# psklavos1/NeRF-Sys

Measured on AMD Instinct MI355X. Metric: rays/sec (train step) + full-image PSNR, 800×800 Lego, 64+128 samples, higher is better.
Workload: dtype f32; 1 GPU; Lego-style 800x800 (synthetic analytic scene, 100 views), 64 coarse + 128 fine hierarchical, 2 x (8x256 MLP), fp32, train step incl. ray gen + Adam [fused engine]; global_batch=4096, rays_per_gpu=4096, parallelism=dp1, precision=fp32, fp32_gemm=split, full=False

## Files before the change

nerf-sys_amd/csrc/gemm_x6.hpp:

```cpp
#pragma once
#include "gemm_bf16.hpp"

typedef float x6_f32x2 __attribute__((ext_vector_type(2)));
typedef __bf16 x6_bf16x2 __attribute__((ext_vector_type(2)));
typedef float x6_f32x4 __attribute__((ext_vector_type(4)));
__device__ __forceinline__ uint32_t x6_pack(float a, float b) {
  return __builtin_bit_cast(uint32_t, __builtin_convertvector(x6_f32x2{a, b}, x6_bf16x2));
}

__device__ __forceinline__ void x6_split4(const float4 v, uint2& h, uint2& m, uint2& l) {
  const uint32_t h0 = x6_pack(v.x, v.y), h1 = x6_pack(v.z, v.w);
  const float r0 = v.x - nerf_bf16_lo(h0), r1 = v.y - nerf_bf16_hi(h0);
  const float r2 = v.z - nerf_bf16_lo(h1), r3 = v.w - nerf_bf16_hi(h1);
  const uint32_t m0 = x6_pack(r0, r1), m1 = x6_pack(r2, r3);
  const uint32_t l0 = x6_pack(r0 - nerf_bf16_lo(m0), r1 - nerf_bf16_hi(m0));
  const uint32_t l1 = x6_pack(r2 - nerf_bf16_lo(m1), r3 - nerf_bf16_hi(m1));
  h = make_uint2(h0, h1);
  m = make_uint2(m0, m1);
  l = make_uint2(l0, l1);
}

__device__ constexpr int X6_PA[6] = {2, 1, 0, 1, 0, 0};
__device__ constexpr int X6_PB[6] = {0, 1, 2, 0, 1, 0};
#define X6_MFMA_BLOCK(acc_, TM_, TN_, FIRST_, SECOND_)                                                      \
  _Pragma("unroll") for (int t_ = 0; t_ < 6; ++t_)                                                        \
    _Pragma("unroll") for (int a_ = 0; a_ < TM_; ++a_)                                                    \
      _Pragma("unroll") for (int b_ = 0; b_ < TN_; ++b_)                                                  \
        acc_[a_][b_] = __builtin_amdgcn_mfma_f32_32x32x16_bf16(FIRST_, SECOND_, acc_[a_][b_], 0, 0, 0);

struct X6Job {
  const float* src;
  nerf_bf16* dst;
  int rows, cols, lds, transpose;
  int64_t plane;
};
struct X6Jobs {
  X6Job j[16];
};
static __global__ void x6_planes_kernel(X6Jobs jobs) {
  const X6Job J = jobs.j[blockIdx.z];
  __shared__ float tile[32][33];
  const int r0 = blockIdx.y * 32, c0 = blockIdx.x * 32;
  if (r0 >= J.rows || c0 >= J.cols) return;
  const int tx = threadIdx.x & 31, ty = threadIdx.x >> 5;
  for (int y = ty; y < 32; y += 8) {
    const int r = r0 + y, c = c0 + tx;
    tile[y][tx] = (r < J.rows && c < J.cols) ? J.src[(int64_t)r * J.lds + c] : 0.f;
  }
  __syncthreads();
  for (int y = ty; y < 32; y += 8) {
    const float v = J.transpose ? tile[tx][y] : tile[y][tx];
    const int orow = J.transpose ? c0 + y : r0 + y, ocol = J.transpose ? r0 + tx : c0 + tx;
    const int orows = J.transpose ? J.cols : J.rows, ocols = J.transpose ? J.rows : J.cols;
    if (orow < orows && ocol < ocols) {
      const nerf_bf16 h = (nerf_bf16)v;
      const float r1 = v - (float)h;
      const nerf_bf16 m = (nerf_bf16)r1;
      const nerf_bf16 l = (nerf_bf16)(r1 - (float)m);
      const int64_t o = (int64_t)orow * ocols + ocol;
      J.dst[o] = h;
      J.dst[J.plane + o] = m;
      J.dst[2 * J.plane + o] = l;
    }
  }
}


constexpr int X6E_PITCH = 36;
constexpr int X6E_WAVE_FLOATS = 32 * X6E_PITCH;
template <int TM, int TN, int EPI>
__device__ __forceinline__ void x6_epilogue_lds(nerf_f32x16 (&acc)[TM][TN], int64_t mw, int n0, int lane,
                                                const float* __restrict__ bias, float* __restrict__ C, int ldc,
                                                const uint32_t* __restrict__ mbits, int ldmb,
                                                uint32_t* __restrict__ mbits_out, float* E) {
  const int li = lane & 31, lh = lane >> 5;
  const int rr = lane >> 3, cc = 4 * (lane & 7);
#pragma unroll
  for (int b = 0; b < TN; ++b) {
    const int nb = n0 + b * 32;
    const int g = nb >> 5;
    float4 bv[4];
#pragma unroll
    for (int q = 0; q < 4; ++q) {
      bv[q] = make_float4(0.f, 0.f, 0.f, 0.f);
      if (EPI == EPI_BIAS || EPI == EPI_BIAS_RELU) bv[q] = *reinterpret_cast<const float4*>(bias + nb + 8 * q + 4 * lh);
    }
#pragma unroll
    for (int a = 0; a < TM; ++a) {
      const int64_t m = mw + a * 32 + li;
      uint32_t word = 0;
      if (EPI == EPI_MASK) word = mbits[m * ldmb + g];
#pragma unroll
      for (int q = 0; q < 4; ++q) {
        float v[4];
#pragma unroll
        for (int e = 0; e < 4; ++e) {
          v[e] = acc[a][b][4 * q + e];
          const float bb = e == 0 ? bv[q].x : (e == 1 ? bv[q].y : (e == 2 ? bv[q].z : bv[q].w));
          if (EPI == EPI_BIAS) v[e] += bb;
          if (EPI == EPI_BIAS_RELU) {
            v[e] = fmaxf(v[e] + bb, 0.f);
            word |= (v[e] > 0.f ? 1u : 0u) << (8 * q + 4 * lh + e);
          }
          if (EPI == EPI_MASK) v[e] = ((word >> (8 * q + 4 * lh + e)) & 1u) ? v[e] : 0.f;
        }
        *reinterpret_cast<float4*>(E + li * X6E_PITCH + 8 * q + 4 * lh) = make_float4(v[0], v[1], v[2], v[3]);
      }
      if (EPI == EPI_BIAS_RELU && mbits_out) {
        word |= __shfl_xor(word, 32, 64);
        if (lh == 0) mbits_out[m * ldmb + g] = word;
      }
      float4 o[4];
#pragma unroll
      for (int i = 0; i < 4; ++i) o[i] = *reinterpret_cast<const float4*>(E + (rr + 8 * i) * X6E_PITCH + cc);
#pragma unroll
      for (int i = 0; i < 4; ++i)
        *reinterpret_cast<float4*>(C + (mw + a * 32 + rr + 8 * i) * ldc + nb + cc) = o[i];
    }
  }
}

template <int EPI, bool BIGSMALL, int NKC, int TN>
__global__ __launch_bounds__(512, 1) void gemm_nt_x6w_kernel(const float* __restrict__ A, int lda,
                                                             const nerf_bf16* __restrict__ Bp, int ldb, int64_t bplane,
                                                             const float* __restrict__ bias, float* __restrict__ C,
                                                             int ldc, const uint32_t* __restrict__ mbits, int ldmb,
                                                             uint32_t* __restrict__ mbits_out, int K, int n_ntiles) {
  constexpr int BK = 32, NW = 8, TM = 1;
  constexpr int WTM = 32 * TM, BM = WTM * NW, BN = 32 * TN;
  constexpr int KS = BK / 16;
  constexpr int LS = BK;
  static_assert(BK == 32, "the swizzle assumes four 16-B chunks per row");
  auto sw = [](int r, int q) { return q ^ ((r >> 2) & 3); };
  constexpr int PL = BN * LS;
  static_assert(2 * 3 * PL >= NW * X6E_WAVE_FLOATS * 2, "epilogue tiles");
  __shared__ __attribute__((aligned(16))) nerf_bf16 smem[2 * 3 * PL];

  const int tile = xcd_remap(blockIdx.x, gridDim.x);
  const int mt = tile / n_ntiles, nt = tile - mt * n_ntiles;
  const int64_t m0 = (int64_t)mt * BM;
  const int n0 = nt * BN;
  const int tid = threadIdx.x, lane = tid & 63, wave = tid >> 6;
  const int li = lane & 31, lh = lane >> 5;
  const nerf_bf16* Bb = Bp + (int64_t)n0 * ldb;
  const float* At = A + (m0 + wave * WTM) * lda;
  int aoff[TM];
#pragma unroll
  for (int a = 0; a < TM; ++a) aoff[a] = (a * 32 + li) * lda + 8 * lh;

  constexpr bool A3 = NKC > 0;
  float4 ra[A3 ? 3 : 2][TM][KS][2];
  constexpr int GPP = BN * BK * 2 / 1024, GPW = 3 * GPP / NW;
  static_assert(GPW * NW == 3 * GPP && GPP * 1024 == BN * BK * 2, "weight staging");
  const int wave_u = __builtin_amdgcn_readfirstlane(tid >> 6);
  const uint32_t gofs = (uint32_t)((((lane >> 2) * ldb) + 8 * ((lane & 3) ^ ((lane >> 4) & 3))) * 2);
  const uint32_t smem_u32 = (uint32_t)(uintptr_t)(const __attribute__((address_space(3))) char*)smem;
#define X6W_ALOAD(set_, k0_)                                                                              \
  _Pragma("unroll") for (int a = 0; a < TM; ++a)                                                         \
    _Pragma("unroll") for (int ks = 0; ks < KS; ++ks)                                                    \
      _Pragma("unroll") for (int hf = 0; hf < 2; ++hf)                                                   \
        ra[set_][a][ks][hf] = *reinterpret_cast<const float4*>(At + aoff[a] + (k0_) + 16 * ks + 4 * hf);
  constexpr int BPG = 2;
#define X6W_BLOAD(k0_, dbuf_)                                                                             \
  {                                                                                                       \
    _Pragma("unroll") for (int a = 0; a < TM; ++a)                                                       \
      _Pragma("unroll") for (int ks = 0; ks < KS; ++ks)                                                  \
        asm volatile("" ::"v"(__builtin_bit_cast(x6_f32x4, ra[j][a][ks][0])),                            \
                     "v"(__builtin_bit_cast(x6_f32x4, ra[j][a][ks][1])) : "memory");                     \
    _Pragma("unroll") for (int i = 0; i < GPW; ++i) {                                                    \
      const int g_ = wave_u + NW * i, p_ = g_ / GPP, rb_ = (g_ % GPP) * 16;                              \
      const nerf_bf16* sb_ = Bb + p_ * bplane + (int64_t)rb_ * ldb + (k0_);                              \
      const uint32_t dst_ = smem_u32 + (uint32_t)((((dbuf_) * 3 + p_) * PL + rb_ * LS) * 2);             \
// ... 129 lines not shown
  constexpr int PG = ((BN + 127) / 128) * 128 + 32, PX = ((BK + 127) / 128) * 128 + 32;
  constexpr int IG = MR * PG, IX = MR * PX;
  constexpr int STAGE = 3 * (IG + IX);
  constexpr int G_F4 = MR * BN / 4, X_F4 = MR * BK / 4;
  constexpr int G_PER = (G_F4 + 255) / 256, X_PER = (X_F4 + 255) / 256;
  __shared__ __attribute__((aligned(16))) nerf_bf16 smem[2 * STAGE];

  const int lin = xcd_remap(blockIdx.x, gridDim.x);
  const int s = lin / n_tiles;
  const int tile = lin - s * n_tiles;
  const int nt = tile / n_ktiles, kt = tile - nt * n_ktiles;
  const int n0 = nt * BN, k0 = kt * BK;
  const int64_t r0 = (int64_t)s * rows_per_split;
  int64_t r1 = r0 + rows_per_split;
  if (r1 > M) r1 = M;
  const int tid = threadIdx.x, lane = tid & 63, wave = tid >> 6;
  const int wn = wave / WAVES_K, wk = wave % WAVES_K;
  const int li = lane & 31, lh = lane >> 5;
  const bool do_bias = (Pb != nullptr) && kt == 0 && wk == 0;

  constexpr int PF = 4;
  float4 rg[PF][G_PER], rx[PF][X_PER];
#define WX6_GLOAD(set_, m_)                                                                                \
  {                                                                                                        \
    _Pragma("unroll") for (int i = 0; i < G_PER; ++i) {                                                    \
      const int f = tid + 256 * i;                                                                         \
      if (G_F4 % 256 == 0 || f < G_F4)                                                                     \
        rg[set_][i] = *reinterpret_cast<const float4*>(G + ((m_) + f / (BN / 4)) * ldg + n0 + (f % (BN / 4)) * 4); \
    }                                                                                                      \
    _Pragma("unroll") for (int i = 0; i < X_PER; ++i) {                                                    \
      const int f = tid + 256 * i;                                                                         \
      if (X_F4 % 256 == 0 || f < X_F4)                                                                     \
        rx[set_][i] = *reinterpret_cast<const float4*>(X + ((m_) + f / (BK / 4)) * ldx + k0 + (f % (BK / 4)) * 4); \
    }                                                                                                      \
  }
#define WX6_SSTORE(set_, buf_)                                                                             \
  {                                                                                                        \
    nerf_bf16* Gs_ = smem + (buf_) * STAGE;                                                                \
    nerf_bf16* Xs_ = Gs_ + 3 * IG;                                                                         \
    _Pragma("unroll") for (int i = 0; i < G_PER; ++i) {                                                    \
      const int f = tid + 256 * i;                                                                         \
      if (G_F4 % 256 == 0 || f < G_F4) {                                                                   \
        uint2 h, m, l;                                                                                     \
        x6_split4(rg[set_][i], h, m, l);                                                                   \
        const int o = (f / (BN / 4)) * PG + (f % (BN / 4)) * 4;                                            \
        *reinterpret_cast<uint2*>(Gs_ + o) = h;                                                            \
        *reinterpret_cast<uint2*>(Gs_ + IG + o) = m;                                                       \
        *reinterpret_cast<uint2*>(Gs_ + 2 * IG + o) = l;                                                   \
      }                                                                                                    \
    }                                                                                                      \
    _Pragma("unroll") for (int i = 0; i < X_PER; ++i) {                                                    \
      const int f = tid + 256 * i;                                                                         \
      if (X_F4 % 256 == 0 || f < X_F4) {                                                                   \
        uint2 h, m, l;                                                                                     \
        x6_split4(rx[set_][i], h, m, l);                                                                   \
        const int o = (f / (BK / 4)) * PX + (f % (BK / 4)) * 4;                                            \
        *reinterpret_cast<uint2*>(Xs_ + o) = h;                                                            \
        *reinterpret_cast<uint2*>(Xs_ + IX + o) = m;                                                       \
        *reinterpret_cast<uint2*>(Xs_ + 2 * IX + o) = l;                                                   \
      }                                                                                                    \
    }                                                                                                      \
  }

  nerf_f32x16 acc[TM][TN];
#pragma unroll
  for (int a = 0; a < TM; ++a)
#pragma unroll
    for (int b = 0; b < TN; ++b)
#pragma unroll
      for (int r = 0; r < 16; ++r) acc[a][b][r] = 0.f;
  float bsum[TM];
#pragma unroll
  for (int a = 0; a < TM; ++a) bsum[a] = 0.f;

  const int grp = lane >> 4, q = (lane >> 2) & 3, p4 = lane & 3;
  const int trow = 8 * (grp >> 1) + q, tcol = 16 * (grp & 1) + 4 * p4;
  auto tr_frag = [&](const nerf_bf16* base, int pitch) {
    const nerf_s16x4 lo = __builtin_amdgcn_ds_read_tr16_b64_v4i16((__attribute__((address_space(3))) nerf_s16x4*)(base));
    const nerf_s16x4 hi =
        __builtin_amdgcn_ds_read_tr16_b64_v4i16((__attribute__((address_space(3))) nerf_s16x4*)(base + 4 * pitch));
    const short v8 __attribute__((ext_vector_type(8))) = {lo[0], lo[1], lo[2], lo[3], hi[0], hi[1], hi[2], hi[3]};
    return __builtin_bit_cast(nerf_bf16x8, v8);
  };

  const int64_t nit = (r1 - r0) / MR;
  if (nit > 0) {
#pragma unroll
    for (int j = 0; j < PF; ++j) WX6_GLOAD(j, r0 + (j < nit ? j : nit - 1) * MR);
    WX6_SSTORE(0, 0);
  }
  __syncthreads();
  for (int64_t it0 = 0; it0 < nit; it0 += PF) {
#pragma unroll
   for (int j = 0; j < PF; ++j) {
    const int64_t it = it0 + j;
    if (it >= nit) break;
    WX6_GLOAD(j, r0 + (it + PF < nit ? it + PF : nit - 1) * MR);
    const nerf_bf16* Gs = smem + (j & 1) * STAGE;
    const nerf_bf16* Xs = Gs + 3 * IG;
    nerf_bf16x8 af[TM][3], bf[TN][3];
#pragma unroll
    for (int pc = 0; pc < 3; ++pc) {
#pragma unroll
      for (int a = 0; a < TM; ++a) af[a][pc] = tr_frag(Gs + pc * IG + trow * PG + wn * WTN + a * 32 + tcol, PG);
#pragma unroll
      for (int b = 0; b < TN; ++b) bf[b][pc] = tr_frag(Xs + pc * IX + trow * PX + wk * WTK + b * 32 + tcol, PX);
    }
    if (do_bias) {
#pragma unroll
      for (int a = 0; a < TM; ++a)
        {
          float t8 = 0.f;
#pragma unroll
          for (int j = 0; j < 8; ++j) t8 += ((float)af[a][0][j] + (float)af[a][1][j]) + (float)af[a][2][j];
          bsum[a] += t8;
        }
    }
    WX6_SSTORE((j + 1) % PF, (j + 1) & 1);
    X6_MFMA_BLOCK(acc, TM, TN, af[a_][X6_PA[t_]], bf[b_][X6_PB[t_]])
#pragma unroll
    for (int q = 0; q < 6 * TM * TN; ++q) {
      __builtin_amdgcn_sched_group_barrier(0x008, 1, 0);
      __builtin_amdgcn_sched_group_barrier(0x002, 5, 0);
      __builtin_amdgcn_sched_group_barrier(0x200, 1, 0);
    }
    __syncthreads();
   }
  }
#undef WX6_GLOAD
#undef WX6_SSTORE

  float* Ps = P + (int64_t)s * slab;
#pragma unroll
  for (int a = 0; a < TM; ++a) {
#pragma unroll
    for (int b = 0; b < TN; ++b) {
      const int k = k0 + wk * WTK + b * 32 + li;
#pragma unroll
      for (int r = 0; r < 16; ++r) {
        const int n = n0 + wn * WTN + a * 32 + (r & 3) + 8 * (r >> 2) + 4 * lh;
        Ps[(int64_t)n * ldp + k] = acc[a][b][r];
      }
    }
  }
  if (do_bias) {
#pragma unroll
    for (int a = 0; a < TM; ++a) {
      const float v = bsum[a] + __shfl_xor(bsum[a], 32, 64);
      if (lh == 0) Pb[(int64_t)s * slab + n0 + wn * WTN + a * 32 + li] = v;
    }
  }
}

__global__ __launch_bounds__(512, 1) void gemm_wgrad_x6w_kernel(const float* __restrict__ G, int ldg,
                                                               const float* __restrict__ X, int ldx,
                                                               float* __restrict__ P, int ldp, float* __restrict__ Pb,
                                                               int64_t slab, int64_t rows_per_split, int64_t M) {
  constexpr int MR = 16, TM = 2, TN = 4, WTN = 64, WTK = 128;
  constexpr int PT = 256 + 32;
  constexpr int IMG = MR * PT;
  constexpr int STAGE = 6 * IMG;
  __shared__ __attribute__((aligned(16))) nerf_bf16 smem[2 * STAGE];

  const int s = blockIdx.x;
  const int64_t r0 = (int64_t)s * rows_per_split;
  int64_t r1 = r0 + rows_per_split;
  if (r1 > M) r1 = M;
  const int tid = threadIdx.x, lane = tid & 63, wave = tid >> 6;
  const int wn = wave >> 1, wk = wave & 1;
  const int li = lane & 31, lh = lane >> 5;
  const bool braw = Pb != nullptr;
  float4 b4 = make_float4(0.f, 0.f, 0.f, 0.f);

  constexpr int PF = 2;
  float4 rg[PF][2], rx[PF][2];
#define WX6W_GLOAD(set_, m_)                                                                               \
  _Pragma("unroll") for (int i = 0; i < 2; ++i) {                                                          \
    const int f = tid + 512 * i;                                                                           \
    rg[set_][i] = *reinterpret_cast<const float4*>(G + ((m_) + (f >> 6)) * ldg + 4 * (f & 63));            \
    rx[set_][i] = *reinterpret_cast<const float4*>(X + ((m_) + (f >> 6)) * ldx + 4 * (f & 63));            \
  }
#define WX6W_SSTORE(set_, buf_)                                                                            \
  _Pragma("unroll") for (int i = 0; i < 2; ++i) {                                                          \
    const int f = tid + 512 * i;                                                                           \
    const int o = (f >> 6) * PT + 4 * (f & 63);                                                            \
    nerf_bf16* S_ = smem + (buf_) * STAGE;                                                                 \
    uint2 h, m, l;                                                                                         \
    x6_split4(rg[set_][i], h, m, l);                                                                       \
    *reinterpret_cast<uint2*>(S_ + o) = h;                                                                 \
    *reinterpret_cast<uint2*>(S_ + IMG + o) = m;                                                           \
    *reinterpret_cast<uint2*>(S_ + 2 * IMG + o) = l;                                                       \
    x6_split4(rx[set_][i], h, m, l);                                                                       \
    *reinterpret_cast<uint2*>(S_ + 3 * IMG + o) = h;                                                       \
    *reinterpret_cast<uint2*>(S_ + 4 * IMG + o) = m;                                                       \
    *reinterpret_cast<uint2*>(S_ + 5 * IMG + o) = l;                                                       \
  }
#define WX6W_BACC(set_, sc_)                                                                               \
  _Pragma("unroll") for (int i = 0; i < 2; ++i) {                                                          \
    b4.x = fmaf(rg[set_][i].x, (sc_), b4.x);                                                               \
    b4.y = fmaf(rg[set_][i].y, (sc_), b4.y);                                                               \
    b4.z = fmaf(rg[set_][i].z, (sc_), b4.z);                                                               \
    b4.w = fmaf(rg[set_][i].w, (sc_), b4.w);                                                               \
  }

  nerf_f32x16 acc[TM][TN];
#pragma unroll
  for (int a = 0; a < TM; ++a)
#pragma unroll
    for (int b = 0; b < TN; ++b)
#pragma unroll
      for (int r = 0; r < 16; ++r) acc[a][b][r] = 0.f;
  const int grp = lane >> 4, q = (lane >> 2) & 3, p4 = lane & 3;
  const int trow = 8 * (grp >> 1) + q, tcol = 16 * (grp & 1) + 4 * p4;
  auto tr_frag = [&](const nerf_bf16* base) {
    const nerf_s16x4 lo = __builtin_amdgcn_ds_read_tr16_b64_v4i16((__attribute__((address_space(3))) nerf_s16x4*)(base));
    const nerf_s16x4 hi =
        __builtin_amdgcn_ds_read_tr16_b64_v4i16((__attribute__((address_space(3))) nerf_s16x4*)(base + 4 * PT));
    const short v8 __attribute__((ext_vector_type(8))) = {lo[0], lo[1], lo[2], lo[3], hi[0], hi[1], hi[2], hi[3]};
    return __builtin_bit_cast(nerf_bf16x8, v8);
  };

  const int64_t nit = (r1 - r0) / MR;
  if (nit > 0) {
#pragma unroll
    for (int j = 0; j < PF; ++j) WX6W_GLOAD(j, r0 + (j < nit ? j : nit - 1) * MR);
    WX6W_SSTORE(0, 0);
    if (braw) WX6W_BACC(0, 1.f);
  }
  __syncthreads();
  auto do_slab = [&](auto J, const int64_t it) __attribute__((always_inline)) {
      constexpr int j = decltype(J)::value;
      WX6W_GLOAD(j, r0 + (it + PF < nit ? it + PF : nit - 1) * MR);
      const int buf = j;
      const nerf_bf16* Gs = smem + buf * STAGE;
      const nerf_bf16* Xs = Gs + 3 * IMG;
      nerf_bf16x8 af[TM][3];
#pragma unroll
      for (int pc = 0; pc < 3; ++pc)
#pragma unroll
        for (int a = 0; a < TM; ++a) af[a][pc] = tr_frag(Gs + pc * IMG + trow * PT + wn * WTN + a * 32 + tcol);
#pragma unroll
      for (int bp = 0; bp < TN / 2; ++bp) {
        if (bp == 1) WX6W_SSTORE((j + 1) % PF, buf ^ 1);
        if (bp == 1 && braw) WX6W_BACC((j + 1) % PF, it + 1 < nit ? 1.f : 0.f);
        nerf_bf16x8 bf[2][3];
#pragma unroll
        for (int pc = 0; pc < 3; ++pc)
#pragma unroll
          for (int b = 0; b < 2; ++b)
            bf[b][pc] = tr_frag(Xs + pc * IMG + trow * PT + wk * WTK + (2 * bp + b) * 32 + tcol);
#pragma unroll
        for (int t = 0; t < 6; ++t)
#pragma unroll
          for (int a = 0; a < TM; ++a)
#pragma unroll
            for (int b = 0; b < 2; ++b)
              acc[a][2 * bp + b] = __builtin_amdgcn_mfma_f32_32x32x16_bf16(af[a][X6_PA[t]], bf[b][X6_PB[t]],
                                                                         acc[a][2 * bp + b], 0, 0, 0);
        if (bp == 1) {
          __builtin_amdgcn_sched_group_barrier(0x100, 6, 0);
#pragma unroll
          for (int q = 0; q < 24; ++q) {
            __builtin_amdgcn_sched_group_barrier(0x008, 1, 0);
            __builtin_amdgcn_sched_group_barrier(0x002, 4, 0);
            if (q & 1) __builtin_amdgcn_sched_group_barrier(0x200, 1, 0);
          }
        }
      }
      __syncthreads();
  };
  int64_t it0 = 0;
  for (; it0 + PF <= nit; it0 += PF) {
    do_slab(std::integral_constant<int, 0>{}, it0);
    do_slab(std::integral_constant<int, 1>{}, it0 + 1);
  }
  if (it0 < nit) do_slab(std::integral_constant<int, 0>{}, it0);
#undef WX6W_GLOAD
#undef WX6W_SSTORE
#undef WX6W_BACC
  if (braw) {
    float* part = reinterpret_cast<float*>(smem);
    *reinterpret_cast<float4*>(part + wave * 256 + 4 * lane) = b4;
    __syncthreads();
    if (tid < 256) {
      float v = part[tid];
#pragma unroll
      for (int w = 1; w < 8; ++w) v += part[w * 256 + tid];
      Pb[(int64_t)s * slab + tid] = v;
    }
  }

  float* Ps = P + (int64_t)s * slab;
#pragma unroll
  for (int a = 0; a < TM; ++a) {
#pragma unroll
    for (int b = 0; b < TN; ++b) {
      const int k = wk * WTK + b * 32 + li;
#pragma unroll
      for (int r = 0; r < 16; ++r) {
        const int n = wn * WTN + a * 32 + (r & 3) + 8 * (r >> 2) + 4 * lh;
        Ps[(int64_t)n * ldp + k] = acc[a][b][r];
      }
    }
  }
}
```

nerf-sys_amd/csrc/mlp.hip:

```cpp
#include "gemm.hpp"
#include "gemm_x6.hpp"
#include "mlp_common.hpp"
#include "mlp_tail.hpp"
#include "mlp_fwd_tail.hpp"

namespace {
using namespace nerf_mlp;

struct WS {
  int64_t Mp;
  float *X3E, *Y[8], *HO, *CIN, *C0;
  uint32_t* MB[8];
  float *dA, *dB, *dO16, *WT, *partial, *partial2;
  float* dZ[8];
  nerf_bf16* WPf;
  nerf_bf16* WPb;
  int S;
  int64_t rps;
  int64_t bytes;
};

constexpr int64_t WT_FLOATS = 7 * 65536;
inline int64_t x6_fwd_off(int i) {
  int64_t o = 0;
// ... 36 lines not shown
    }
    w.dO16 = take(Mp * 16);
    w.WT = take(WT_FLOATS);
    w.WPb = reinterpret_cast<nerf_bf16*>(take(X6_BWD_BF16 / 2));
    w.S = n_splits(Mp);
    w.rps = round_up(nerf_cdiv(Mp, w.S), 64);
    w.partial = take((int64_t)w.S * layout().total);
    w.partial2 = take((int64_t)(TAIL_NQ - 1) * w.S * (layout().total - P2BASE));
  }
  w.bytes = (int64_t)((char*)p - (char*)base);
  return w;
}

inline int ld_of(const WS& w, int i) { return (i == 3) ? 320 : 256; }


constexpr int PE_TP = 33;
__global__ __launch_bounds__(256) void pe_xyz_kernel(const float* __restrict__ xd, int64_t M, int64_t Mp,
                                                     float* __restrict__ X3E) {
  __shared__ float tile[4][64 * PE_TP];
  const int lane = threadIdx.x & 63, wv = threadIdx.x >> 6;
  const int64_t m0 = ((int64_t)blockIdx.x * 4 + wv) * 64;
  if (m0 >= Mp) return;
  const int64_t m = m0 + lane;
  float v[64];
#pragma unroll
  for (int c = 0; c < 64; ++c) v[c] = 0.f;
  if (m < M) {
    const float x[3] = {xd[m * 6], xd[m * 6 + 1], xd[m * 6 + 2]};
#pragma unroll
    for (int k = 0; k < 3; ++k) {
      v[k] = x[k];
      float band = 1.0f;
#pragma unroll
      for (int l = 0; l < 10; ++l) {
        float s, c;
        sincosf(x[k] * band, &s, &c);
        v[3 + k * 20 + l] = c;
        v[3 + k * 20 + 10 + l] = s;
        band *= 2.0f;
      }
    }
  }
  float* t = tile[wv];
#pragma unroll
  for (int hf = 0; hf < 2; ++hf) {
#pragma unroll
    for (int c = 0; c < 32; ++c) t[lane * PE_TP + c] = v[32 * hf + c];
    __builtin_amdgcn_fence(__ATOMIC_RELEASE, "wavefront");
    __builtin_amdgcn_wave_barrier();
    __builtin_amdgcn_fence(__ATOMIC_ACQUIRE, "wavefront");
#pragma unroll
    for (int i = 0; i < 8; ++i) {
      const int r = 8 * i + (lane >> 3), q = lane & 7;
      const float* src = t + r * PE_TP + 4 * q;
      *reinterpret_cast<float4*>(X3E + (m0 + r) * 320 + 256 + 32 * hf + 4 * q) =
          make_float4(src[0], src[1], src[2], src[3]);
    }
    __builtin_amdgcn_fence(__ATOMIC_RELEASE, "wavefront");
    __builtin_amdgcn_wave_barrier();
    __builtin_amdgcn_fence(__ATOMIC_ACQUIRE, "wavefront");
  }
}

struct TJob {
  const float* src;
  float* dst;
  int rows, cols, lds;
};
struct TJobs {
  TJob j[10];
};
__global__ void transpose_kernel(TJobs jobs) {
  const TJob J = jobs.j[blockIdx.z];
  __shared__ float tile[32][33];
  const int r0 = blockIdx.y * 32, c0 = blockIdx.x * 32;
  if (r0 >= J.rows || c0 >= J.cols) return;
  const int tx = threadIdx.x & 31, ty = threadIdx.x >> 5;
  for (int y = ty; y < 32; y += 8) {
    const int r = r0 + y, c = c0 + tx;
    tile[y][tx] = (r < J.rows && c < J.cols) ? J.src[(int64_t)r * J.lds + c] : 0.f;
  }
  __syncthreads();
  for (int y = ty; y < 32; y += 8) {
    const int c = c0 + y, r = r0 + tx;
    if (c < J.cols && r < J.rows) J.dst[(int64_t)c * J.rows + r] = tile[tx][y];
  }
}


#ifndef NERF_NT16_MINW
#define NERF_NT16_MINW 3
#endif

template <int EPI>
int nt(const float* A, int lda, const float* B, int ldb, const float* bias, float* C, int ldc, const uint32_t* mbits,
       uint32_t* mbits_out, int64_t M, int N, int K, hipStream_t st) {
  if (M % 128 || N != 256 || K % 16) return NERF_E_ARG;
  const int ntn = N / 128;
  gemm_nt16_kernel<128, 128, 2, EPI, NERF_NT16_MINW><<<(unsigned)((M / 128) * ntn), 256, 0, st>>>(
      A, lda, B, ldb, bias, C, ldc, mbits, N / 32, mbits_out, K, ntn);
  return NERF_OK;
}

int wgrad(const float* G, int ldg, const float* X, int ldx, int tensor_w, const WS& w, int N, int K, hipStream_t st) {
  const Layout& L = layout();
  float* P = w.partial + L.off[tensor_w];
  float* Pb = w.partial + L.off[tensor_w + 1];
  const int ldp = L.cols[tensor_w];
  const int64_t slab = L.total;
  if (N != 256) return NERF_E_ARG;
  auto t128 = [&](const float* Xk, float* Pk, float* Pbk) {
    gemm_wgrad_kernel<128, 128, 2><<<4 * w.S, 256, 0, st>>>(G, ldg, Xk, ldx, Pk, ldp, Pbk, slab, w.rps, w.Mp, 2, 4);
  };
  auto t64 = [&](const float* Xk, float* Pk, float* Pbk) {
    gemm_wgrad_kernel<64, 64, 2, 32><<<4 * w.S, 256, 0, st>>>(G, ldg, Xk, ldx, Pk, ldp, Pbk, slab, w.rps, w.Mp, 1, 4);
  };
  if (K == 64) {
    t64(X, P, Pb);
  } else if (K == 256) {
    t128(X, P, Pb);
  } else if (K == 320) {
    t128(X, P, Pb);
    t64(X + 256, P + 256, nullptr);
  } else {
    return NERF_E_ARG;
  }
  return NERF_OK;
}

template <int EPI>
int nt_x6(const float* A, int lda, const nerf_bf16* Bp, int ldb, int64_t bplane, const float* bias, float* C, int ldc,
          const uint32_t* mbits, uint32_t* mbits_out, int64_t M, int N, int K, hipStream_t st) {
  static_assert(EPI == EPI_BIAS_RELU || EPI == EPI_MASK, "trunk forward or input gradient");
  if (M % 256 || N != 256 || lda % 4 || ldb % 8) return NERF_E_ARG;
  if constexpr (EPI == EPI_MASK) {
    if (K != 256) return NERF_E_ARG;
    gemm_nt_x6w_kernel<EPI, true, 8, 4><<<(unsigned)((M / 256) * 2), 512, 0, st>>>(A, lda, Bp, ldb, bplane, bias, C, ldc,
                                                                                   mbits, N / 32, mbits_out, K, 2);
  } else {
    if (K % 64) return NERF_E_ARG;
    gemm_nt_x6w_kernel<EPI, false, 0, 8><<<(unsigned)(M / 256), 512, 0, st>>>(A, lda, Bp, ldb, bplane, bias, C, ldc,
                                                                              mbits, N / 32, mbits_out, K, 1);
  }
  return NERF_OK;
}

int wgrad_x6(const float* G, int ldg, const float* X, int ldx, int tensor_w, const WS& w, int N, int K, hipStream_t st) {
  const Layout& L = layout();
  float* P = w.partial + L.off[tensor_w];
  float* Pb = w.partial + L.off[tensor_w + 1];
  const int ldp = L.cols[tensor_w];
  const int64_t slab = L.total;
  if (N != 256 || ldg % 4 || ldx % 4) return NERF_E_ARG;
  auto t128 = [&](const float* Xk, float* Pk, float* Pbk) {
    gemm_wgrad_x6w_kernel<<<w.S, 512, 0, st>>>(G, ldg, Xk, ldx, Pk, ldp, Pbk, slab, w.rps, w.Mp);
  };
  auto t64 = [&](const float* Xk, float* Pk, float* Pbk) {
    gemm_wgrad_x6_kernel<128, 64, 4><<<2 * w.S, 256, 0, st>>>(G, ldg, Xk, ldx, Pk, ldp, Pbk, slab, w.rps, w.Mp, 1, 2);
  };
  if (K == 64) {
    t64(X, P, Pb);
  } else if (K == 256) {
    t128(X, P, Pb);
  } else if (K == 320) {
    t128(X, P, Pb);
    t64(X + 256, P + 256, nullptr);
  } else {
    return NERF_E_ARG;
  }
  return NERF_OK;
}

}

extern "C" int64_t nerf_mlp_layout(int64_t* table) {
  const Layout& L = layout();
  if (table) {
    for (int t = 0; t < NT; ++t) {
      table[4 * t + 0] = L.off[t];
      table[4 * t + 1] = L.rows[t];
      table[4 * t + 2] = L.cols[t];
      table[4 * t + 3] = L.creal[t];
    }
  }
  return L.total;
}

extern "C" int64_t nerf_mlp_workspace_bytes(int64_t M, int training) {
  if (M < 0) return -1;
  return carve(nullptr, M, training).bytes + 256;
}

extern "C" int nerf_mlp_fwd_ex(const float* w, const float* x_d, int64_t M, float* rgb_sigma, void* ws,
                               int64_t ws_bytes, int training, int flags, hipEvent_t* ev, hipStream_t st) {
  NERF_CHECK_ARG(w && ws && M >= 0 && (M == 0 || (x_d && rgb_sigma)));
  if (flags & ~NERF_MLP_NATIVE_FP32) return NERF_E_ENUM;
  const bool native = flags & NERF_MLP_NATIVE_FP32;
  if (!nerf_aligned16(w) || !nerf_aligned16(ws) || !nerf_aligned16(rgb_sigma)) return NERF_E_ALIGN;
  const WS W = carve(ws, M, training);
  if (ws_bytes < W.bytes) return NERF_E_WORKSPACE;
  if (M == 0) return NERF_OK;
  const Layout& L = layout();
  const int64_t Mp = W.Mp;
  auto Wt = [&](int t) { return w + L.off[t]; };

  pe_xyz_kernel<<<(unsigned)nerf_cdiv(Mp, 256), 256, 0, st>>>(x_d, M, Mp, W.X3E);
  if (!native) {
    X6Jobs jobs{};
    for (int i = 0; i < 8; ++i)
      jobs.j[i] = X6Job{Wt(2 * i), W.WPf + x6_fwd_off(i), 256, KPAD[i], KPAD[i], 0, 256 * (int64_t)KPAD[i]};
    x6_planes_kernel<<<dim3(10, 8, 8), 256, 0, st>>>(jobs);
  }
  const float* in = W.X3E + 256;
  int ld_in = 320;
  for (int i = 0; i < 8; ++i) {
    float* out = W.Y[i];
    const int ld_out = training ? ld_of(W, i) : ((i % 2 == 0) ? 256 : 320);
    if (i == 4) { in = W.X3E; ld_in = 320; }
    if (ev) (void)hipEventRecord(ev[2 * i], st);
    if (native)
      TRY(nt<EPI_BIAS_RELU>(in, ld_in, Wt(2 * i), KPAD[i], Wt(2 * i + 1), out, ld_out, nullptr,
                            training ? W.MB[i] : nullptr, Mp, 256, KPAD[i], st));
    else
      TRY(nt_x6<EPI_BIAS_RELU>(in, ld_in, W.WPf + x6_fwd_off(i), KPAD[i], 256 * (int64_t)KPAD[i], Wt(2 * i + 1), out,
                               ld_out, nullptr, training ? W.MB[i] : nullptr, Mp, 256, KPAD[i], st));
    if (ev) (void)hipEventRecord(ev[2 * i + 1], st);
    in = out;
    ld_in = ld_out;
  }
  {
    FwdTailArgs T{};
    T.Y7 = in; T.ldy = ld_in; T.xd = x_d; T.w = w;
    T.off_wh = L.off[16]; T.off_bh = L.off[17]; T.off_wc0 = L.off[18]; T.off_bc0 = L.off[19];
    T.off_wc1 = L.off[20]; T.off_bc1 = L.off[21];
    T.HO = W.HO; T.CIN = W.CIN; T.C0 = W.C0; T.out = rgb_sigma;
    T.M = M; T.Mp = Mp; T.ntiles = (int)(Mp / FT_ROWS);
    const int n_cu = nerf_cu_count();
    const int grid = T.ntiles < 2 * n_cu ? T.ntiles : 2 * n_cu;
    if (training)
      fwd_tail_kernel<true><<<grid, 256, 0, st>>>(T);
    else
      fwd_tail_kernel<false><<<grid, 256, 0, st>>>(T);
  }
  return nerf_launch_status();
}


extern "C" int nerf_mlp_fwd(const float* w, const float* x_d, int64_t M, float* rgb_sigma, void* ws, int64_t ws_bytes,
                            int training, hipEvent_t* ev, hipStream_t st) {
  return nerf_mlp_fwd_ex(w, x_d, M, rgb_sigma, ws, ws_bytes, training, 0, ev, st);
}

extern "C" int64_t nerf_mlp_workspace_bytes_2s(int64_t M) {
  if (M < 0) return -1;
  return carve(nullptr, M, 2).bytes + 256;
}

namespace {
int mlp_bwd_impl(const float* w, int64_t M, const float* d_rgb_sigma, float* d_w, int accumulate, void* ws,
                 int64_t ws_bytes, int flags, hipEvent_t* ev, hipStream_t st, hipStream_t stw, hipEvent_t* sync) {
  NERF_CHECK_ARG(w && d_w && ws && M >= 0 && (M == 0 || d_rgb_sigma));
  NERF_CHECK_ARG(!stw || sync);
  if (flags & ~(NERF_MLP_NATIVE_FP32 | NERF_MLP_NATIVE_DGRAD)) return NERF_E_ENUM;
  const bool native = flags & NERF_MLP_NATIVE_FP32;
  const bool split_dgrad = !native && !(flags & NERF_MLP_NATIVE_DGRAD);
  if (!nerf_aligned16(w) || !nerf_aligned16(ws) || !nerf_aligned16(d_w) || !nerf_aligned16(d_rgb_sigma))
    return NERF_E_ALIGN;
  const bool two = stw != nullptr;
  const WS W = carve(ws, M, two ? 2 : 1);
  if (ws_bytes < W.bytes) return NERF_E_WORKSPACE;
  hipStream_t sw = two ? stw : st;
  auto handoff = [&](int k) -> int {
    if (!two) return NERF_OK;
    hipError_t e = hipEventRecord(sync[k], st);
    if (e == hipSuccess) e = hipStreamWaitEvent(stw, sync[k], 0);
    return nerf_hip_status(e);
  };
  const Layout& L = layout();
  if (M == 0) {
    if (!accumulate) (void)hipMemsetAsync(d_w, 0, L.total * sizeof(float), st);
    return nerf_launch_status();
  }
  const int64_t Mp = W.Mp;
  auto Wt = [&](int t) { return w + L.off[t]; };

  float* T = W.WT;
  float* WTi[8] = {nullptr};
  TJobs jobs{};
  int nj = 0;
  if (!split_dgrad) {
    for (int i = 1; i < 8; ++i) {
      WTi[i] = T;
      jobs.j[nj++] = TJob{Wt(2 * i), T, 256, 256, KPAD[i]};
      T += 65536;
    }
  } else {
    X6Jobs xj{};
    for (int i = 1; i < 8; ++i)
      xj.j[i - 1] = X6Job{Wt(2 * i), W.WPb + 3 * 65536 * (int64_t)(i - 1), 256, 256, KPAD[i], 1, 65536};
    x6_planes_kernel<<<dim3(8, 8, 7), 256, 0, st>>>(xj);
  }
  if (nj) transpose_kernel<<<dim3(8, 8, nj), 256, 0, st>>>(jobs);

  float* dcur = W.dA;
  float* dnext = W.dB;
  if (ev) (void)hipEventRecord(ev[2], st);
  color_bwd_kernel<float, float><<<TAIL_NQ * W.S, 256, 0, st>>>(d_rgb_sigma, W.HO, W.C0, W.CIN, Wt(18), Wt(20), W.dO16,
                                                          W.partial, L.total, L.off[18], L.off[19], L.off[20], L.off[21],
                                                          W.rps, M, Mp, W.partial2, L.total - P2BASE, P2BASE, 16);
  head_bwd_kernel<<<TAIL_NQ * W.S, 256, 0, st>>>(W.dO16, W.Y[7], Wt(16), dcur, W.partial, L.total, W.partial2,
                                           L.total - P2BASE, P2BASE, L.off[16], L.off[17], W.rps, Mp);
  if (ev) (void)hipEventRecord(ev[3], st);
  TRY(handoff(1));
  for (int i = 7; i >= 0; --i) {
    const float* X = (i == 0) ? W.X3E + 256 : (i == 4 ? W.X3E : W.Y[i - 1]);
    const int ldx = (i == 0 || i == 4) ? 320 : ld_of(W, i - 1);
    if (two && i < 7) TRY(handoff(8 - i));
    if (ev) (void)hipEventRecord(ev[4 * i], sw);
    if (native)
// ... 50 lines not shown
```

Measured before the change: 248,000 rays/s.

## Fuse K=320 weight-gradient into one x6 kernel with extra 64-column tile

The 320-wide weight gradient (the skip layer with 64 encoding columns) was computed by two launches: the 256-column wide kernel plus a separate 64-column kernel that re-read G. A template parameter KX now lets the wide kernel load the 64 extra X columns, split them into bf16 triplets in a wider LDS image, and accumulate them in an extra accumulator per wave. This removes one launch and the second pass over G. It also adds precomputed LDS/global offset pointers with asm barriers and moves the next-slab global prefetch to after the first MFMA half. The cost is more LDS, more registers, and extra MFMAs concentrated in the bp==0 half, which may unbalance the schedule.

```diff
diff --git a/nerf-sys_amd/csrc/gemm_x6.hpp b/nerf-sys_amd/csrc/gemm_x6.hpp
--- a/nerf-sys_amd/csrc/gemm_x6.hpp
+++ b/nerf-sys_amd/csrc/gemm_x6.hpp
@@ -18,6 +18,12 @@
   h = make_uint2(h0, h1);
   m = make_uint2(m0, m1);
   l = make_uint2(l0, l1);
+}
+__device__ __forceinline__ void x6_split2(const float2 v, uint32_t& h, uint32_t& m, uint32_t& l) {
+  h = x6_pack(v.x, v.y);
+  const float r0 = v.x - nerf_bf16_lo(h), r1 = v.y - nerf_bf16_hi(h);
+  m = x6_pack(r0, r1);
+  l = x6_pack(r0 - nerf_bf16_lo(m), r1 - nerf_bf16_hi(m));
 }
 
 __device__ constexpr int X6_PA[6] = {2, 1, 0, 1, 0, 0};
@@ -453,14 +459,19 @@
   }
 }
 
+template <int KX>
 __global__ __launch_bounds__(512, 1) void gemm_wgrad_x6w_kernel(const float* __restrict__ G, int ldg,
                                                                const float* __restrict__ X, int ldx,
                                                                float* __restrict__ P, int ldp, float* __restrict__ Pb,
                                                                int64_t slab, int64_t rows_per_split, int64_t M) {
+  static_assert(KX == 0 || KX == 64, "extra X columns: none, or trunk.4's 64 encoding columns");
   constexpr int MR = 16, TM = 2, TN = 4, WTN = 64, WTK = 128;
   constexpr int PT = 256 + 32;
-  constexpr int IMG = MR * PT;
-  constexpr int STAGE = 6 * IMG;
+  constexpr int PX = KX ? 256 + KX + 96 : PT;
+  static_assert((PT * 2) % 256 == 64 && (PX * 2) % 256 == 64 && PX >= 256 + KX, "image pitch");
+  constexpr int IMG = MR * PT, IMX = MR * PX;
+  constexpr int STAGE = 3 * (IMG + IMX);
+  static_assert(2 * STAGE * 2 <= 160 * 1024 && 2 * STAGE * 2 >= 8 * 256 * 4, "LDS: two stages; the bias partials");
   __shared__ __attribute__((aligned(16))) nerf_bf16 smem[2 * STAGE];
 
   const int s = blockIdx.x;
@@ -475,26 +486,56 @@
 
   constexpr int PF = 2;
   float4 rg[PF][2], rx[PF][2];
+  float2 rxe[PF];
+  typedef const __attribute__((address_space(1))) char* gl_ptr;
+  typedef const __attribute__((address_space(1))) x6_f32x4* gl_f4;
+  typedef const __attribute__((address_space(1))) x6_f32x2* gl_f2;
+  const unsigned gofs = 4u * ((tid >> 6) * ldg + 4 * (tid & 63)), xofs = 4u * ((tid >> 6) * ldx + 4 * (tid & 63));
+  const unsigned eofs = 4u * ((tid >> 5) * ldx + 256 + 2 * (tid & 31));
 #define WX6W_GLOAD(set_, m_)                                                                               \
-  _Pragma("unroll") for (int i = 0; i < 2; ++i) {                                                          \
-    const int f = tid + 512 * i;                                                                           \
-    rg[set_][i] = *reinterpret_cast<const float4*>(G + ((m_) + (f >> 6)) * ldg + 4 * (f & 63));            \
-    rx[set_][i] = *reinterpret_cast<const float4*>(X + ((m_) + (f >> 6)) * ldx + 4 * (f & 63));            \
+  if constexpr (KX > 0) {                                                                                  \
+    gl_ptr Gm_ = (gl_ptr)(G + (m_) * ldg), Xm_ = (gl_ptr)(X + (m_) * ldx);                                 \
+    gl_ptr Gm8_ = Gm_ + (int64_t)ldg * 32, Xm8_ = Xm_ + (int64_t)ldx * 32;                                 \
+    unsigned go_ = gofs, xo_ = xofs, eo_ = eofs;                                                           \
+    asm volatile("" : "+s"(Gm_), "+s"(Xm_), "+s"(Gm8_), "+s"(Xm8_), "+v"(go_), "+v"(xo_), "+v"(eo_));      \
+    rg[set_][0] = __builtin_bit_cast(float4, *(gl_f4)(Gm_ + go_));                                         \
+    rx[set_][0] = __builtin_bit_cast(float4, *(gl_f4)(Xm_ + xo_));                                         \
+    rg[set_][1] = __builtin_bit_cast(float4, *(gl_f4)(Gm8_ + go_));                                        \
+    rx[set_][1] = __builtin_bit_cast(float4, *(gl_f4)(Xm8_ + xo_));                                        \
+    rxe[set_] = __builtin_bit_cast(float2, *(gl_f2)(Xm_ + eo_));                                           \
+  } else {                                                                                                 \
+    _Pragma("unroll") for (int i = 0; i < 2; ++i) {                                                        \
+      const int f = tid + 512 * i;                                                                         \
+      rg[set_][i] = *reinterpret_cast<const float4*>(G + ((m_) + (f >> 6)) * ldg + 4 * (f & 63));          \
+      rx[set_][i] = *reinterpret_cast<const float4*>(X + ((m_) + (f >> 6)) * ldx + 4 * (f & 63));          \
+    }                                                                                                      \
   }
 #define WX6W_SSTORE(set_, buf_)                                                                            \
-  _Pragma("unroll") for (int i = 0; i < 2; ++i) {                                                          \
-    const int f = tid + 512 * i;                                                                           \
-    const int o = (f >> 6) * PT + 4 * (f & 63);                                                            \
+  {                                                                                                        \
     nerf_bf16* S_ = smem + (buf_) * STAGE;                                                                 \
-    uint2 h, m, l;                                                                                         \
-    x6_split4(rg[set_][i], h, m, l);                                                                       \
-    *reinterpret_cast<uint2*>(S_ + o) = h;                                                                 \
-    *reinterpret_cast<uint2*>(S_ + IMG + o) = m;                                                           \
-    *reinterpret_cast<uint2*>(S_ + 2 * IMG + o) = l;                                                       \
-    x6_split4(rx[set_][i], h, m, l);                                                                       \
-    *reinterpret_cast<uint2*>(S_ + 3 * IMG + o) = h;                                                       \
-    *reinterpret_cast<uint2*>(S_ + 4 * IMG + o) = m;                                                       \
-    *reinterpret_cast<uint2*>(S_ + 5 * IMG + o) = l;                                                       \
+    _Pragma("unroll") for (int i = 0; i < 2; ++i) {                                                        \
+      const int f = tid + 512 * i;                                                                         \
+      const int o = (f >> 6) * PT + 4 * (f & 63);                                                          \
+      nerf_bf16* dg_ = (nerf_bf16*)wrG + 8 * i * PT;                                                       \
+      nerf_bf16* dx_ = (nerf_bf16*)wrX + 8 * i * PX;                                                       \
+      uint2 h, m, l;                                                                                       \
+      x6_split4(rg[set_][i], h, m, l);                                                                     \
+      *reinterpret_cast<uint2*>(KX ? dg_ : S_ + o) = h;                                                    \
+      *reinterpret_cast<uint2*>(KX ? dg_ + IMG : S_ + IMG + o) = m;                                        \
+      *reinterpret_cast<uint2*>(KX ? dg_ + 2 * IMG : S_ + 2 * IMG + o) = l;                                \
+      x6_split4(rx[set_][i], h, m, l);                                                                     \
+      *reinterpret_cast<uint2*>(KX ? dx_ : S_ + 3 * IMG + o) = h;                                          \
+      *reinterpret_cast<uint2*>(KX ? dx_ + IMX : S_ + 4 * IMG + o) = m;                                    \
+      *reinterpret_cast<uint2*>(KX ? dx_ + 2 * IMX : S_ + 5 * IMG + o) = l;                                \
+    }                                                                                                      \
+    if constexpr (KX > 0) {                                                                                \
+      nerf_bf16* de_ = (nerf_bf16*)wrE;                                                                    \
+      uint32_t h, m, l;                                                                                    \
+      x6_split2(rxe[set_], h, m, l);                                                                       \
+      *reinterpret_cast<uint32_t*>(de_) = h;                                                               \
+      *reinterpret_cast<uint32_t*>(de_ + IMX) = m;                                                         \
+      *reinterpret_cast<uint32_t*>(de_ + 2 * IMX) = l;                                                     \
+    }                                                                                                      \
   }
 #define WX6W_BACC(set_, sc_)                                                                               \
   _Pragma("unroll") for (int i = 0; i < 2; ++i) {                                                          \
@@ -511,53 +552,92 @@
     for (int b = 0; b < TN; ++b)
 #pragma unroll
       for (int r = 0; r < 16; ++r) acc[a][b][r] = 0.f;
+  nerf_f32x16 accx[TM];
+  if constexpr (KX > 0) {
+#pragma unroll
+    for (int a = 0; a < TM; ++a)
+#pragma unroll
+      for (int r = 0; r < 16; ++r) accx[a][r] = 0.f;
+  }
   const int grp = lane >> 4, q = (lane >> 2) & 3, p4 = lane & 3;
   const int trow = 8 * (grp >> 1) + q, tcol = 16 * (grp & 1) + 4 * p4;
-  auto tr_frag = [&](const nerf_bf16* base) {
+  auto tr_frag = [&](const nerf_bf16* base, const int pitch) {
     const nerf_s16x4 lo = __builtin_amdgcn_ds_read_tr16_b64_v4i16((__attribute__((address_space(3))) nerf_s16x4*)(base));
     const nerf_s16x4 hi =
-        __builtin_amdgcn_ds_read_tr16_b64_v4i16((__attribute__((address_space(3))) nerf_s16x4*)(base + 4 * PT));
+        __builtin_amdgcn_ds_read_tr16_b64_v4i16((__attribute__((address_space(3))) nerf_s16x4*)(base + 4 * pitch));
     const short v8 __attribute__((ext_vector_type(8))) = {lo[0], lo[1], lo[2], lo[3], hi[0], hi[1], hi[2], hi[3]};
     return __builtin_bit_cast(nerf_bf16x8, v8);
   };
 
-  const int64_t nit = (r1 - r0) / MR;
+  typedef __attribute__((address_space(3))) nerf_bf16* lds_ptr;
+  lds_ptr rdG = nullptr, rdX = nullptr, rdE = nullptr, wrG = nullptr, wrX = nullptr, wrE = nullptr;
+#define WX6W_MOVE(rd_, wr_)                                                                                \
+  {                                                                                                        \
+    rdG += (rd_); rdX += (rd_); rdE += (rd_); wrG += (wr_); wrX += (wr_); wrE += (wr_);                    \
+    asm volatile("" : "+v"(rdG), "+v"(rdX), "+v"(rdE), "+v"(wrG), "+v"(wrX), "+v"(wrE));                   \
+  }
+  if constexpr (KX > 0) {
+    const lds_ptr sm = (lds_ptr)smem;
+    rdG = sm + trow * PT + wn * WTN + tcol;
+    rdX = sm + 3 * IMG + trow * PX + wk * WTK + tcol;
+    rdE = sm + 3 * IMG + trow * PX + 256 + 32 * wk + tcol;
+    wrG = sm + (tid >> 6) * PT + 4 * (tid & 63);
+    wrX = sm + 3 * IMG + (tid >> 6) * PX + 4 * (tid & 63);
+    wrE = sm + 3 * IMG + (tid >> 5) * PX + 256 + 2 * (tid & 31);
+    WX6W_MOVE(0, 0);
+  }
+  typedef typename std::conditional<KX != 0, int, int64_t>::type it_t;
+  const it_t nit = (it_t)((r1 - r0) / MR);
   if (nit > 0) {
 #pragma unroll
     for (int j = 0; j < PF; ++j) WX6W_GLOAD(j, r0 + (j < nit ? j : nit - 1) * MR);
     WX6W_SSTORE(0, 0);
     if (braw) WX6W_BACC(0, 1.f);
   }
+  if constexpr (KX > 0) WX6W_MOVE(0, STAGE);
   __syncthreads();
-  auto do_slab = [&](auto J, const int64_t it) __attribute__((always_inline)) {
+  auto do_slab = [&](auto J, const it_t it) __attribute__((always_inline)) {
       constexpr int j = decltype(J)::value;
-      WX6W_GLOAD(j, r0 + (it + PF < nit ? it + PF : nit - 1) * MR);
+      if constexpr (KX == 0) WX6W_GLOAD(j, r0 + (it + PF < nit ? it + PF : nit - 1) * MR);
       const int buf = j;
       const nerf_bf16* Gs = smem + buf * STAGE;
       const nerf_bf16* Xs = Gs + 3 * IMG;
+      const nerf_bf16* Ga = (const nerf_bf16*)rdG, * Xa = (const nerf_bf16*)rdX, * Ea = (const nerf_bf16*)rdE;
       nerf_bf16x8 af[TM][3];
 #pragma unroll
       for (int pc = 0; pc < 3; ++pc)
 #pragma unroll
-        for (int a = 0; a < TM; ++a) af[a][pc] = tr_frag(Gs + pc * IMG + trow * PT + wn * WTN + a * 32 + tcol);
+        for (int a = 0; a < TM; ++a)
+          af[a][pc] = tr_frag(KX ? Ga + pc * IMG + a * 32 : Gs + pc * IMG + trow * PT + wn * WTN + a * 32 + tcol, PT);
 #pragma unroll
       for (int bp = 0; bp < TN / 2; ++bp) {
         if (bp == 1) WX6W_SSTORE((j + 1) % PF, buf ^ 1);
         if (bp == 1 && braw) WX6W_BACC((j + 1) % PF, it + 1 < nit ? 1.f : 0.f);
-        nerf_bf16x8 bf[2][3];
+        nerf_bf16x8 bf[2][3], bfx[3];
 #pragma unroll
         for (int pc = 0; pc < 3; ++pc)
 #pragma unroll
           for (int b = 0; b < 2; ++b)
-            bf[b][pc] = tr_frag(Xs + pc * IMG + trow * PT + wk * WTK + (2 * bp + b) * 32 + tcol);
-#pragma unroll
-        for (int t = 0; t < 6; ++t)
+            bf[b][pc] = tr_frag(KX ? Xa + pc * IMX + (2 * bp + b) * 32
+                                   : Xs + pc * IMG + trow * PT + wk * WTK + (2 * bp + b) * 32 + tcol, PX);
+        if (KX > 0 && bp == 0) {
+#pragma unroll
+          for (int pc = 0; pc < 3; ++pc) bfx[pc] = tr_frag(Ea + pc * IMX, PX);
+        }
+#pragma unroll
+        for (int t = 0; t < 6; ++t) {
 #pragma unroll
           for (int a = 0; a < TM; ++a)
 #pragma unroll
             for (int b = 0; b < 2; ++b)
               acc[a][2 * bp + b] = __builtin_amdgcn_mfma_f32_32x32x16_bf16(af[a][X6_PA[t]], bf[b][X6_PB[t]],
                                                                          acc[a][2 * bp + b], 0, 0, 0);
+          if (KX > 0 && bp == 0) {
+#pragma unroll
+            for (int a = 0; a < TM; ++a)
+              accx[a] = __builtin_amdgcn_mfma_f32_32x32x16_bf16(af[a][X6_PA[t]], bfx[X6_PB[t]], accx[a], 0, 0, 0);
+          }
+        }
         if (bp == 1) {
           __builtin_amdgcn_sched_group_barrier(0x100, 6, 0);
 #pragma unroll
@@ -567,10 +647,14 @@
             if (q & 1) __builtin_amdgcn_sched_group_barrier(0x200, 1, 0);
           }
         }
-      }
+        if constexpr (KX > 0) {
+          if (bp == 0) WX6W_GLOAD(j, r0 + (it + PF < nit ? it + PF : nit - 1) * MR);
+        }
+      }
+      if constexpr (KX > 0) WX6W_MOVE(j == 0 ? STAGE : -STAGE, j == 0 ? -STAGE : STAGE);
       __syncthreads();
   };
-  int64_t it0 = 0;
+  it_t it0 = 0;
   for (; it0 + PF <= nit; it0 += PF) {
     do_slab(std::integral_constant<int, 0>{}, it0);
     do_slab(std::integral_constant<int, 1>{}, it0 + 1);
@@ -579,15 +663,20 @@
 #undef WX6W_GLOAD
 #undef WX6W_SSTORE
 #undef WX6W_BACC
+#undef WX6W_MOVE
+  int te = tid;
+  if constexpr (KX > 0) asm volatile("" : "+v"(te));
+  const int elane = KX ? te & 63 : lane, ewave = KX ? te >> 6 : wave, ewn = KX ? ewave >> 1 : wn, ewk = KX ? ewave & 1 : wk;
+  const int eli = KX ? elane & 31 : li, elh = KX ? elane >> 5 : lh;
   if (braw) {
     float* part = reinterpret_cast<float*>(smem);
-    *reinterpret_cast<float4*>(part + wave * 256 + 4 * lane) = b4;
+    *reinterpret_cast<float4*>(part + ewave * 256 + 4 * elane) = b4;
     __syncthreads();
-    if (tid < 256) {
-      float v = part[tid];
-#pragma unroll
-      for (int w = 1; w < 8; ++w) v += part[w * 256 + tid];
-      Pb[(int64_t)s * slab + tid] = v;
+    if (te < 256) {
+      float v = part[te];
+#pragma unroll
+      for (int w = 1; w < 8; ++w) v += part[w * 256 + te];
+      Pb[(int64_t)s * slab + te] = v;
     }
   }
 
@@ -596,12 +685,20 @@
   for (int a = 0; a < TM; ++a) {
 #pragma unroll
     for (int b = 0; b < TN; ++b) {
-      const int k = wk * WTK + b * 32 + li;
+      const int k = ewk * WTK + b * 32 + eli;
 #pragma unroll
       for (int r = 0; r < 16; ++r) {
-        const int n = wn * WTN + a * 32 + (r & 3) + 8 * (r >> 2) + 4 * lh;
+        const int n = ewn * WTN + a * 32 + (r & 3) + 8 * (r >> 2) + 4 * elh;
         Ps[(int64_t)n * ldp + k] = acc[a][b][r];
       }
     }
+    if constexpr (KX > 0) {
+      const int k = 256 + 32 * ewk + eli;
+#pragma unroll
+      for (int r = 0; r < 16; ++r) {
+        const int n = ewn * WTN + a * 32 + (r & 3) + 8 * (r >> 2) + 4 * elh;
+        Ps[(int64_t)n * ldp + k] = accx[a][r];
+      }
+    }
   }
 }
diff --git a/nerf-sys_amd/csrc/mlp.hip b/nerf-sys_amd/csrc/mlp.hip
--- a/nerf-sys_amd/csrc/mlp.hip
+++ b/nerf-sys_amd/csrc/mlp.hip
@@ -212,20 +212,13 @@
   float* Pb = w.partial + L.off[tensor_w + 1];
   const int ldp = L.cols[tensor_w];
   const int64_t slab = L.total;
-  if (N != 256 || ldg % 4 || ldx % 4) return NERF_E_ARG;
-  auto t128 = [&](const float* Xk, float* Pk, float* Pbk) {
-    gemm_wgrad_x6w_kernel<<<w.S, 512, 0, st>>>(G, ldg, Xk, ldx, Pk, ldp, Pbk, slab, w.rps, w.Mp);
-  };
-  auto t64 = [&](const float* Xk, float* Pk, float* Pbk) {
-    gemm_wgrad_x6_kernel<128, 64, 4><<<2 * w.S, 256, 0, st>>>(G, ldg, Xk, ldx, Pk, ldp, Pbk, slab, w.rps, w.Mp, 1, 2);
-  };
+  if (N != 256 || ldg % 4 || ldx % 4 || ldx < K || ldp < K) return NERF_E_ARG;
   if (K == 64) {
-    t64(X, P, Pb);
+    gemm_wgrad_x6_kernel<128, 64, 4><<<2 * w.S, 256, 0, st>>>(G, ldg, X, ldx, P, ldp, Pb, slab, w.rps, w.Mp, 1, 2);
   } else if (K == 256) {
-    t128(X, P, Pb);
+    gemm_wgrad_x6w_kernel<0><<<w.S, 512, 0, st>>>(G, ldg, X, ldx, P, ldp, Pb, slab, w.rps, w.Mp);
   } else if (K == 320) {
-    t128(X, P, Pb);
-    t64(X + 256, P + 256, nullptr);
+    gemm_wgrad_x6w_kernel<64><<<w.S, 512, 0, st>>>(G, ldg, X, ldx, P, ldp, Pb, slab, w.rps, w.Mp);
   } else {
     return NERF_E_ARG;
   }
```

Measured after the change: 249,900 rays/s, median of 6. No clear change (+0.8%).
